# zhaowenlan1779/hekaton-system

Measured on AMD Instinct MI355X. Metric: subcircuit Groth16 proofs/sec (whole node), big-merkle, higher is better.
Workload: dtype u32 limbs (Montgomery mod-p integers)

## Files before the change

### __graft_entry__.py

```python
import os
import subprocess
import sys

ROOT = os.path.dirname(os.path.abspath(__file__))
if ROOT not in sys.path:
    sys.path.insert(0, ROOT)


def build():
    csrc = os.path.join(ROOT, "hekaton_system_amd", "csrc")
    jobs = str(min(8, os.cpu_count() or 1))
    subprocess.check_call(["make", "-C", csrc, "-j", jobs, "ARCH=gfx950"])
    subprocess.check_call(["make", "-C", csrc, "check", "ARCH=gfx950"], stdout=subprocess.DEVNULL)
    subprocess.check_call(["make", "-C", os.path.join(ROOT, "apps")], stdout=subprocess.DEVNULL)
    subprocess.check_call(["make", "-C", os.path.join(ROOT, "tests", "device_shim"), "-j", "2", "ARCH=gfx950"],
                          stdout=subprocess.DEVNULL)
    from oracle import c_oracle
    c_oracle.build()
    import hekaton_system_amd
    from hekaton_system_amd import capi
    lib = capi.load()
    for sym in capi.EXPORTS:
        getattr(lib, sym)


def smoke():
    import numpy as np
    from hekaton_system_amd import capi
    from tests import golden_util as gu
    case = gu.load("groth16.json")["bn254"][0]
    pk = case["pk"]
    with capi.Context("bn254", 0) as ctx:
        dpk = ctx.pk_upload(
            a_g=gu.hb(pk["a_g"]), b_g=gu.hb(pk["b_g"]), b_h=gu.hb(pk["b_h"]), h_g=gu.hb(pk["h_g"]),
            ck_stages=[gu.hb(c) for c in pk["ck"]], deltas_g=gu.hb(pk["deltas_g"]),
            last_delta_h=gu.hb(pk["last_delta_h"]), alpha_g=gu.hb(pk["alpha_g"]), beta_g=gu.hb(pk["beta_g"]),
            beta_h=gu.hb(pk["beta_h"]), matrices=(gu.csr(case["A"]), gu.csr(case["B"]), gu.csr(case["C"])),
            n_inst=case["n_inst"], n_constraints=case["n_constraints"])
        z = gu.hb(case["z_mont"])
        fr = ctx.fr_bytes
        s0, e0 = case["stage_ranges"][0]
        w0 = z[(case["n_inst"] + s0) * fr:(case["n_inst"] + e0) * fr]
        kap = gu.hb(case["kappas_mont"])
        com = dpk.commit(0, w0, kap[:fr])
        assert com.tobytes().hex() == case["comms"][0], "commitment differs from oracle"
        a, b, c = dpk.prove(z, gu.hb(case["r_mont"]), gu.hb(case["s_mont"]), kap)
        got = (a.tobytes().hex(), b.tobytes().hex(), c.tobytes().hex())
        want = (case["proof"]["a"], case["proof"]["b"], case["proof"]["c"])
        assert got == want, "proof differs from oracle"
        dpk.free()
    print("smoke ok: commit + prove on cuda:0 match the oracle bit for bit")


if __name__ == "__main__":
    build()
    print("build ok")
```

### hekaton_system_amd/csrc/ntt.cuh

```cuda
#pragma once
#include "field.cuh"

namespace hk {

constexpr int NTT_TILE_LOG = 11;
constexpr int NTT_THREADS = 512;
constexpr int POW_TABLE_BITS = 11;
constexpr int POW_TABLE_SIZE = 1 << POW_TABLE_BITS;

#if defined(__HIPCC__)

template <class Fr>
__device__ __forceinline__ Fr fr_load(const Fr* p) {
    Fr r;
    const uint4* s = reinterpret_cast<const uint4*>(p);
    uint4 a = s[0], b = s[1];
    r.v[0] = a.x; r.v[1] = a.y; r.v[2] = a.z; r.v[3] = a.w;
    r.v[4] = b.x; r.v[5] = b.y; r.v[6] = b.z; r.v[7] = b.w;
    return r;
}
template <class Fr>
__device__ __forceinline__ void fr_store(Fr* p, const Fr& lazy) {
    Fr r = Fr::canon(lazy);
    uint4* d = reinterpret_cast<uint4*>(p);
    d[0] = make_uint4(r.v[0], r.v[1], r.v[2], r.v[3]);
    d[1] = make_uint4(r.v[4], r.v[5], r.v[6], r.v[7]);
}

template <class Fr>
__global__ void k_pow_table(Fr* __restrict__ tw, const Fr* __restrict__ sq, u32 count, u32 nbits) {
    u32 i = blockIdx.x * blockDim.x + threadIdx.x;
    if (i >= count) return;
    Fr acc = Fr::one();
    for (u32 k = 0; k < nbits; k++)
        if ((i >> k) & 1) acc = Fr::mul(acc, fr_load(&sq[k]));
    fr_store(&tw[i], acc);
}

template <class Fr>
__device__ __forceinline__ Fr pow_from_tables(const Fr* __restrict__ pw, u32 j, u32 logn) {
    Fr g = fr_load(&pw[j & (POW_TABLE_SIZE - 1)]);
    if (logn > POW_TABLE_BITS) g = Fr::mul(g, fr_load(&pw[POW_TABLE_SIZE + ((j >> POW_TABLE_BITS) & (POW_TABLE_SIZE - 1))]));
    if (logn > 2 * POW_TABLE_BITS) g = Fr::mul(g, fr_load(&pw[2 * POW_TABLE_SIZE + (j >> (2 * POW_TABLE_BITS))]));
    return g;
}

template <class Fr>
__global__ void k_stage_tables(Fr* __restrict__ tws, const Fr* __restrict__ tw, u32 log_table) {
    size_t i = (size_t)blockIdx.x * blockDim.x + threadIdx.x;
    if ((i + 1) >> log_table) return;
    u32 s = 31 - __clz((u32)(i + 1));
    size_t j = i + 1 - ((size_t)1 << s);
    fr_store(&tws[i], fr_load(&tw[j << (log_table - s - 1)]));
}

template <class Fr, int DIT>
__global__ void __launch_bounds__(NTT_THREADS)
k_ntt_pass4(Fr* __restrict__ data, size_t stride_vec, const Fr* __restrict__ tws, u32 logn, u32 lo, u32 nst,
            u32 cols_bits, int post, u32 npost, Fr scale, const Fr* __restrict__ pw, const Fr* __restrict__ sub,
            Fr kc) {
    extern __shared__ uint4 lds_raw[];
    Fr* lds = reinterpret_cast<Fr*>(lds_raw);
    const u32 nthr = blockDim.x;
    if (blockIdx.y >= npost) post = 0;
    Fr* vec = data + (size_t)blockIdx.y * stride_vec;
    const u32 cols = 1u << cols_bits;
    const u32 tile_elems = 1u << (nst + cols_bits);
    const u32 mid_bits = lo - cols_bits;
    const u32 mid = blockIdx.x & ((1u << mid_bits) - 1u);
    const size_t base = ((size_t)(blockIdx.x >> mid_bits) << (lo + nst)) | ((size_t)mid << cols_bits);
    for (u32 e = threadIdx.x; e < tile_elems; e += nthr) {
        u32 r = e >> cols_bits, c = e & (cols - 1);
        lds[e] = fr_load(&vec[base | ((size_t)r << lo) | c]);
    }
    __syncthreads();
    const u32 npair = nst >> 1;
    for (u32 k = 0; k < npair; k++) {
        const u32 l = DIT ? 2 * k : nst - 2 - 2 * k;
        const u32 s = lo + l;
        const Fr* t_lo = tws + (((size_t)1 << s) - 1);
        const Fr* t_hi = tws + (((size_t)2 << s) - 1);
        for (u32 q = threadIdx.x; q < (tile_elems >> 2); q += nthr) {
            u32 c = q & (cols - 1), rr = q >> cols_bits;
            u32 r0 = ((rr >> l) << (l + 2)) | (rr & ((1u << l) - 1u));
            u32 j = (u32)((base | ((size_t)r0 << lo) | c) & (((size_t)1 << s) - 1));
            Fr wc = fr_load(&t_lo[j]);
            Fr wa = fr_load(&t_hi[j]);
            Fr wb = fr_load(&t_hi[j + (1u << s)]);
            u32 i0 = (r0 << cols_bits) | c, st = 1u << (l + cols_bits);
            Fr x0 = lds[i0], x1 = lds[i0 + st], x2 = lds[i0 + 2 * st], x3 = lds[i0 + 3 * st];
            if (DIT) {
                Fr v = Fr::mul(x1, wc), u = Fr::mul(x3, wc);
                x1 = Fr::sub(x0, v); x0 = Fr::add(x0, v);
                x3 = Fr::sub(x2, u); x2 = Fr::add(x2, u);
                v = Fr::mul(x2, wa); u = Fr::mul(x3, wb);
                x2 = Fr::sub(x0, v); x0 = Fr::add(x0, v);
                x3 = Fr::sub(x1, u); x1 = Fr::add(x1, u);
            } else {
                Fr v = Fr::sub(x0, x2), u = Fr::sub(x1, x3);
                x0 = Fr::add(x0, x2); x1 = Fr::add(x1, x3);
                x2 = Fr::mul(v, wa); x3 = Fr::mul(u, wb);
                v = Fr::sub(x0, x1); u = Fr::sub(x2, x3);
                x0 = Fr::add(x0, x1); x2 = Fr::add(x2, x3);
                x1 = Fr::mul(v, wc); x3 = Fr::mul(u, wc);
            }
            lds[i0] = x0; lds[i0 + st] = x1; lds[i0 + 2 * st] = x2; lds[i0 + 3 * st] = x3;
        }
        __syncthreads();
    }
    if (nst & 1) {
        const u32 l = DIT ? nst - 1 : 0;
        const u32 s = lo + l;
        const Fr* t_lo = tws + (((size_t)1 << s) - 1);
        for (u32 q = threadIdx.x; q < (tile_elems >> 1); q += nthr) {
            u32 c = q & (cols - 1), rr = q >> cols_bits;
            u32 r0 = ((rr >> l) << (l + 1)) | (rr & ((1u << l) - 1u));
            u32 j = (u32)((base | ((size_t)r0 << lo) | c) & (((size_t)1 << s) - 1));
            Fr w = fr_load(&t_lo[j]);
            u32 i0 = (r0 << cols_bits) | c, st = 1u << (l + cols_bits);
            Fr x0 = lds[i0], x1 = lds[i0 + st];
            if (DIT) {
                Fr v = Fr::mul(x1, w);
                lds[i0] = Fr::add(x0, v);
                lds[i0 + st] = Fr::sub(x0, v);
            } else {
                lds[i0] = Fr::add(x0, x1);
                lds[i0 + st] = Fr::mul(Fr::sub(x0, x1), w);
            }
        }
        __syncthreads();
    }
    for (u32 e = threadIdx.x; e < tile_elems; e += nthr) {
        u32 r = e >> cols_bits, c = e & (cols - 1);
        size_t gi = base | ((size_t)r << lo) | c;
        Fr x = lds[e];
        if (post & 2) x = Fr::mul(x, pow_from_tables(pw, logn ? (__brev((u32)gi) >> (32 - logn)) : 0u, logn));
        if (post & 4) x = Fr::sub(x, Fr::mul(fr_load(&sub[gi]), kc));
        if (post & 1) x = Fr::mul(x, scale);
        fr_store(&vec[gi], x);
    }
}

template <class Fr>
__global__ void k_scale_pow(Fr* __restrict__ data, size_t stride_vec, const Fr* __restrict__ pw, Fr scale,
                            u32 logn, int bitrev_index, int use_pow) {
    size_t pos = (size_t)blockIdx.x * blockDim.x + threadIdx.x;
    if (pos >> logn) return;
    Fr* vec = data + (size_t)blockIdx.y * stride_vec;
    Fr x = fr_load(&vec[pos]);
    x = Fr::mul(x, scale);
    if (use_pow) {
        u32 j = bitrev_index ? (logn ? (__brev((u32)pos) >> (32 - logn)) : 0u) : (u32)pos;
        x = Fr::mul(x, pow_from_tables(pw, j, logn));
    }
    fr_store(&vec[pos], x);
}

template <class Fr>
__global__ void k_bitrev(Fr* __restrict__ data, u32 logn) {
    size_t pos = (size_t)blockIdx.x * blockDim.x + threadIdx.x;
    if (pos >> logn) return;
    u32 r = logn ? (__brev((u32)pos) >> (32 - logn)) : 0u;
    if (r > pos) {
        Fr a = fr_load(&data[pos]), b = fr_load(&data[r]);
        fr_store(&data[pos], b);
        fr_store(&data[r], a);
    }
}

template <class Fr>
__global__ void k_mul_pointwise(Fr* __restrict__ a, const Fr* __restrict__ b, size_t m) {
    size_t i = (size_t)blockIdx.x * blockDim.x + threadIdx.x;
    if (i >= m) return;
    fr_store(&a[i], Fr::mul(fr_load(&a[i]), fr_load(&b[i])));
}

#endif

}
```

### hekaton_system_amd/csrc/ntt_host.cuh

```cuda
#pragma once
#include "curve_ops_impl.cuh"
#include "ntt.cuh"
#include "ntt_plan.h"
#include "csr.cuh"

namespace hk {

template <class Fr>
static Fr host_halve(const Fr& a) {
    u32 t[Fr::N + 1];
    u64 c = 0;
    bool odd = a.v[0] & 1;
    for (int i = 0; i < Fr::N; i++) {
        c += (u64)a.v[i] + (odd ? Fr::Params::MOD[i] : 0u);
        t[i] = (u32)c;
        c >>= 32;
    }
    t[Fr::N] = (u32)c;
    Fr r;
    for (int i = 0; i < Fr::N; i++) r.v[i] = (t[i] >> 1) | (t[i + 1] << 31);
    return r;
}
template <class Fr>
static Fr host_from_limbs(const u32* l) {
    Fr r;
    for (int i = 0; i < Fr::N; i++) r.v[i] = l[i];
    return r;
}

struct NttTables {
    std::mutex mu;
    u32 log_table = 0;
    void* tw_fwd = nullptr;
    void* tw_inv = nullptr;
    void* pw_g = nullptr;
    void* pw_ginv = nullptr;
    std::vector<void*> retired;
};

template <class C>
struct NttHost {
    typedef typename C::Fr Fr;

    static hk_status ensure(hk_ctx* ctx, u32 log_m, NttTables** out) {
        if (log_m > C::TWO_ADICITY) return HK_ERR_DOMAIN_TOO_LARGE;
        std::unique_lock<std::mutex> lk(ctx->mu);
        if (!ctx->ntt) ctx->ntt = new NttTables();
        NttTables* T = ctx->ntt;
        lk.unlock();
        std::unique_lock<std::mutex> tl(T->mu);
        *out = T;
        if (T->log_table >= log_m && T->tw_fwd) return HK_OK;
        u32 L = log_m < 16 ? 16 : log_m;
        if (L > C::TWO_ADICITY) L = C::TWO_ADICITY;
        HK_HIP(hipSetDevice(ctx->device));
        std::vector<Fr> sq(32), sqi(32);
        Fr w = host_from_limbs<Fr>(C::ROOT);
        for (u32 k = 0; k < C::TWO_ADICITY - L; k++) w = Fr::sqr(w);
        Fr winv = Fr::one();
        for (u32 k = 0; k < L; k++) {
            sq[k] = w;
            winv = Fr::mul(winv, w);
            w = Fr::sqr(w);
        }
        Fr t = winv;
        for (u32 k = 0; k < L; k++) { sqi[k] = t; t = Fr::sqr(t); }
        const u32 NG = 3 * POW_TABLE_BITS;
        std::vector<Fr> gs(NG), gis(NG);
        Fr g = host_from_limbs<Fr>(C::GEN), gi = host_from_limbs<Fr>(C::GEN_INV);
        for (u32 k = 0; k < NG; k++) { gs[k] = g; gis[k] = gi; g = Fr::sqr(g); gi = Fr::sqr(gi); }
        Fr *d_sq = nullptr, *tmp = nullptr, *tf = nullptr, *ti = nullptr, *pg = nullptr, *pgi = nullptr;
        size_t half = (size_t)1 << (L - 1), full = (size_t)1 << L;
        HK_HIP(hipMalloc((void**)&d_sq, sizeof(Fr) * (64 + 2 * NG)));
        HK_HIP(hipMalloc((void**)&tmp, sizeof(Fr) * half));
        HK_HIP(hipMalloc((void**)&tf, sizeof(Fr) * full));
        HK_HIP(hipMalloc((void**)&ti, sizeof(Fr) * full));
        HK_HIP(hipMalloc((void**)&pg, sizeof(Fr) * 3 * POW_TABLE_SIZE));
        HK_HIP(hipMalloc((void**)&pgi, sizeof(Fr) * 3 * POW_TABLE_SIZE));
        HK_HIP(hipMemcpy(d_sq, sq.data(), sizeof(Fr) * 32, hipMemcpyHostToDevice));
        HK_HIP(hipMemcpy(d_sq + 32, sqi.data(), sizeof(Fr) * 32, hipMemcpyHostToDevice));
        HK_HIP(hipMemcpy(d_sq + 64, gs.data(), sizeof(Fr) * NG, hipMemcpyHostToDevice));
        HK_HIP(hipMemcpy(d_sq + 64 + NG, gis.data(), sizeof(Fr) * NG, hipMemcpyHostToDevice));
        u32 blocks = (u32)((half + 255) / 256), blocks_full = (u32)((full + 255) / 256);
        hipLaunchKernelGGL((k_pow_table<Fr>), dim3(blocks), dim3(256), 0, 0, tmp, d_sq, (u32)half, L - 1);
        hipLaunchKernelGGL((k_stage_tables<Fr>), dim3(blocks_full), dim3(256), 0, 0, tf, tmp, L);
        hipLaunchKernelGGL((k_pow_table<Fr>), dim3(blocks), dim3(256), 0, 0, tmp, d_sq + 32, (u32)half, L - 1);
        hipLaunchKernelGGL((k_stage_tables<Fr>), dim3(blocks_full), dim3(256), 0, 0, ti, tmp, L);
        for (u32 lvl = 0; lvl < 3; lvl++) {
            hipLaunchKernelGGL((k_pow_table<Fr>), dim3(POW_TABLE_SIZE / 256), dim3(256), 0, 0, pg + POW_TABLE_SIZE * lvl,
                               d_sq + 64 + POW_TABLE_BITS * lvl, (u32)POW_TABLE_SIZE, (u32)POW_TABLE_BITS);
            hipLaunchKernelGGL((k_pow_table<Fr>), dim3(POW_TABLE_SIZE / 256), dim3(256), 0, 0, pgi + POW_TABLE_SIZE * lvl,
                               d_sq + 64 + NG + POW_TABLE_BITS * lvl, (u32)POW_TABLE_SIZE, (u32)POW_TABLE_BITS);
        }
        HK_HIP(hipGetLastError());
        HK_HIP(hipDeviceSynchronize());
        HK_HIP(hipFree(d_sq));
        HK_HIP(hipFree(tmp));
        for (void* p : {T->tw_fwd, T->tw_inv, T->pw_g, T->pw_ginv})
            if (p) T->retired.push_back(p);
        T->tw_fwd = tf; T->tw_inv = ti; T->pw_g = pg; T->pw_ginv = pgi;
        T->log_table = L;
        return HK_OK;
    }

    static Fr size_inv(u32 log_m) {
        Fr x = Fr::one();
        for (u32 k = 0; k < log_m; k++) x = host_halve(x);
        return x;
    }
    static Fr vanishing_inv_on_coset(u32 log_m) {
        Fr g = host_from_limbs<Fr>(C::GEN);
        for (u32 k = 0; k < log_m; k++) g = Fr::sqr(g);
        return fp_inv(Fr::sub(g, Fr::one()));
    }

    struct Post {
        int post = 0;
        u32 nvec = 0xffffffffu;
        const Fr* scale = nullptr;
        const Fr* pw = nullptr;
        const Fr* sub = nullptr;
        const Fr* kc = nullptr;
    };

    static hk_status passes(hipStream_t s, Fr* data, size_t stride, u32 batch, u32 logn, const Fr* tws, int dit,
                            const Post& ep = Post()) {
        if (logn == 0) return HK_OK;
        static const u32 tile_log = [] {
            const char* e = getenv("HK_NTT_TILE_LOG");
            return ntt_plan_tile_log(e ? (u32)atoi(e) : NTT_PLAN_TILE_LOG);
        }();
        static const u32 upper_max = [] {
            const char* e = getenv("HK_NTT_UPPER_MAX");
            return ntt_plan_upper_max(e ? (u32)atoi(e) : NTT_PLAN_UPPER_MAX, tile_log);
        }();
        const u32 threads = 1u << (tile_log - 2);
        NttPass ps[NTT_PLAN_MAX_PASSES];
        int np = ntt_pass_plan(logn, tile_log, upper_max, ps);
        Fr one = Fr::one();
        for (int k = 0; k < np; k++) {
            const NttPass& p = dit ? ps[k] : ps[np - 1 - k];
            u32 tile_log = p.nst + p.cols_bits;
            dim3 grid(1u << (logn - tile_log), batch);
            size_t lds = sizeof(Fr) << tile_log;
            bool last = k == np - 1;
            int pp = last ? ep.post : 0;
            const Fr& sc = (pp & 1) ? *ep.scale : one;
            const Fr& kc = (pp & 4) ? *ep.kc : one;
            if (dit)
                hipLaunchKernelGGL((k_ntt_pass4<Fr, 1>), grid, dim3(threads), lds, s, data, stride, tws, logn, p.lo,
                                   p.nst, p.cols_bits, pp, ep.nvec, sc, ep.pw, ep.sub, kc);
            else
                hipLaunchKernelGGL((k_ntt_pass4<Fr, 0>), grid, dim3(threads), lds, s, data, stride, tws, logn, p.lo,
                                   p.nst, p.cols_bits, pp, ep.nvec, sc, ep.pw, ep.sub, kc);
        }
        HK_HIP(hipGetLastError());
        return HK_OK;
    }

    static hk_status scale(hipStream_t s, Fr* data, size_t stride, u32 batch, u32 logn, const Fr* pw,
                           const Fr& sc, int bitrev_index, int use_pow) {
        size_t n = (size_t)1 << logn;
        hipLaunchKernelGGL((k_scale_pow<Fr>), dim3((u32)((n + 255) / 256), batch), dim3(256), 0, s, data,
                           stride, pw, sc, logn, bitrev_index, use_pow);
        HK_HIP(hipGetLastError());
        return HK_OK;
    }
    static hk_status bitrev(hipStream_t s, Fr* data, u32 logn) {
        size_t n = (size_t)1 << logn;
        hipLaunchKernelGGL((k_bitrev<Fr>), dim3((u32)((n + 255) / 256)), dim3(256), 0, s, data, logn);
        HK_HIP(hipGetLastError());
        return HK_OK;
    }
};

template <class C>
hk_status Ops<C>::ntt(hk_ctx* ctx, void* data, unsigned log_m, int inverse, int coset) {
    typedef NttHost<C> N;
    NttTables* T;
    HK_TRY(N::ensure(ctx, log_m, &T));
    LaneGuard g(ctx);
    Lane* L = g.lane;
    if (!L) return HK_ERR_DEVICE;
    size_t n = (size_t)1 << log_m;
    Fr* stage;
    HK_TRY(L->carve([&](Carve& c) { stage = c.n<Fr>(n); }));
    bool dev = is_device_ptr(data);
    Fr* d = (Fr*)data;
    if (!dev) {
        d = stage;
        HK_HIP(hipMemcpyAsync(d, data, n * sizeof(Fr), hipMemcpyHostToDevice, L->stream));
    }
    hipStream_t s = L->stream;
    if (!inverse) {
        if (coset) HK_TRY(N::scale(s, d, n, 1, log_m, (const Fr*)T->pw_g, Fr::one(), 0, 1));
        HK_TRY(N::passes(s, d, n, 1, log_m, (const Fr*)T->tw_fwd, 0));
        HK_TRY(N::bitrev(s, d, log_m));
    } else {
        Fr minv = N::size_inv(log_m);
        typename N::Post ep;
        ep.post = coset ? 3 : 1;
        ep.scale = &minv;
        ep.pw = (const Fr*)T->pw_ginv;
        HK_TRY(N::passes(s, d, n, 1, log_m, (const Fr*)T->tw_inv, 0, ep));
        HK_TRY(N::bitrev(s, d, log_m));
    }
    if (!dev) HK_HIP(hipMemcpyAsync(data, d, n * sizeof(Fr), hipMemcpyDeviceToHost, s));
    return L->settle();
}

template <class C>
struct QapHost {
    typedef typename C::Fr Fr;
    typedef NttHost<C> N;

    static u32 domain_log(size_t n_c, size_t n_inst) {
        size_t need = n_c + n_inst;
        u32 lg = 0;
        while (((size_t)1 << lg) < need) lg++;
        return lg;
    }
    static hk_status run(hipStream_t s, NttTables* T, const CsrDev& A, const CsrDev& B, const CsrDev& Cm,
                         size_t n_inst, size_t n_c, const Fr* z, Fr* abc, u32 log_m) {
        size_t m = (size_t)1 << log_m;
        const CsrDev* Ms[3] = {&A, &B, &Cm};
        for (int k = 0; k < 3; k++) {
            hipLaunchKernelGGL((k_spmv<Fr>), dim3((u32)((m + 255) / 256)), dim3(256), 0, s,
                               Ms[k]->row_ptr, Ms[k]->col, (const Fr*)Ms[k]->val, z, abc + k * m,
                               (u32)n_c, k == 0 ? (u32)n_inst : 0u, (u32)m);
        }
        const Fr* tinv = (const Fr*)T->tw_inv;
        const Fr* tfwd = (const Fr*)T->tw_fwd;
        typename N::Post e1;
        e1.post = 2;
        e1.nvec = 2;
        e1.pw = (const Fr*)T->pw_g;
        HK_TRY(N::passes(s, abc, m, 3, log_m, tinv, 0, e1));
        HK_TRY(N::passes(s, abc, m, 2, log_m, tfwd, 1));
        hipLaunchKernelGGL((k_mul_pointwise<Fr>), dim3((u32)((m + 255) / 256)), dim3(256), 0, s, abc, abc + m, m);
        Fr minv = N::size_inv(log_m);
        Fr mm = fp_inv(Fr::mul(minv, minv));
        Fr k = Fr::mul(N::vanishing_inv_on_coset(log_m), Fr::mul(minv, Fr::mul(minv, minv)));
        typename N::Post e2;
        e2.post = 2 | 4 | 1;
        e2.pw = (const Fr*)T->pw_ginv;
        e2.sub = abc + 2 * m;
        e2.kc = &mm;
        e2.scale = &k;
        HK_TRY(N::passes(s, abc, m, 1, log_m, tinv, 0, e2));
        HK_HIP(hipGetLastError());
        return HK_OK;
    }
};

template <class C>
hk_status Ops<C>::witness_map(hk_ctx* ctx, const hk_csr* A, const hk_csr* B, const hk_csr* Cm, size_t n_inst,
                              size_t n_c, const void* z, size_t n_v, void* h_out, size_t h_cap,
                              size_t* m_out) {
    typedef QapHost<C> Q;
    if (A->n_rows != n_c || B->n_rows != n_c || Cm->n_rows != n_c || n_inst > n_v || n_inst < 1) return HK_ERR_ARG;
    if (!csr_host_ok(A) || !csr_host_ok(B) || !csr_host_ok(Cm)) return HK_ERR_ARG;
    u32 log_m = Q::domain_log(n_c, n_inst);
    if (log_m > C::TWO_ADICITY) return HK_ERR_DOMAIN_TOO_LARGE;
    size_t m = (size_t)1 << log_m;
    if (m_out) *m_out = m;
    if (h_cap < m) return HK_ERR_LEN;
    NttTables* T;
    HK_TRY(NttHost<C>::ensure(ctx, log_m, &T));
    R1csStage stage(A, B, Cm, n_v, sizeof(Fr));
    Staged zin = staged(z, n_v * sizeof(Fr));
    LaneGuard g(ctx);
    Lane* L = g.lane;
    if (!L) return HK_ERR_DEVICE;
    Fr* abc;
    HK_TRY(L->carve([&](Carve& c) {
        stage.carve(c);
        stage_carve(c, &zin, 1);
        abc = c.n<Fr>(3 * m);
    }));
    CsrDev D[3];
    HK_TRY(stage.upload(L, D));
    HK_TRY(stage_upload(L, &zin, 1));
    HK_TRY(Q::run(L->stream, T, D[0], D[1], D[2], n_inst, n_c, (const Fr*)zin.p, abc, log_m));
    HK_TRY(NttHost<C>::bitrev(L->stream, abc, log_m));
    HK_HIP(hipMemcpyAsync(h_out, abc, m * sizeof(Fr),
                          is_device_ptr(h_out) ? hipMemcpyDeviceToDevice : hipMemcpyDeviceToHost, L->stream));
    return L->settle();
}

template <class C>
void Ops<C>::ctx_release(hk_ctx* ctx) {
    for (auto& e : ctx->fb_cache)
        if (e.table) (void)hipFree(e.table);
    ctx->fb_cache.clear();
    if (!ctx->ntt) return;
    NttTables* T = ctx->ntt;
    for (void* p : {T->tw_fwd, T->tw_inv, T->pw_g, T->pw_ginv})
        if (p) (void)hipFree(p);
    for (void* p : T->retired) (void)hipFree(p);
    delete T;
    ctx->ntt = nullptr;
}

}
```

Baseline: 126.3.

## Precompute coset twist tables and special-case trivial-twiddle NTT stages

Adds cached per-size coset twist tables in bit-reversed order. The post-NTT coset multiply becomes a single table load instead of up to three pow-table loads and two multiplies, and the quotient scale is folded into the inverse table and the subtraction constant. It also reorders the odd radix-2 stage and adds specialised s==0 radix-4/radix-2 butterflies that skip twiddle loads and multiplies by one. The trade-offs are two extra m-sized device tables per domain size, a one-time build with a stream sync, and more branching in the NTT kernel.

```diff
diff --git a/__graft_entry__.py b/__graft_entry__.py
--- a/__graft_entry__.py
+++ b/__graft_entry__.py
@@ -15,6 +15,8 @@
     subprocess.check_call(["make", "-C", os.path.join(ROOT, "apps")], stdout=subprocess.DEVNULL)
     subprocess.check_call(["make", "-C", os.path.join(ROOT, "tests", "device_shim"), "-j", "2", "ARCH=gfx950"],
                           stdout=subprocess.DEVNULL)
+    subprocess.check_call(["make", "-C", os.path.join(ROOT, "tests", "device_shim"), "-f", "twist.mk", "-j", "2",
+                           "ARCH=gfx950"], stdout=subprocess.DEVNULL)
     from oracle import c_oracle
     c_oracle.build()
     import hekaton_system_amd
diff --git a/hekaton_system_amd/csrc/ntt.cuh b/hekaton_system_amd/csrc/ntt.cuh
--- a/hekaton_system_amd/csrc/ntt.cuh
+++ b/hekaton_system_amd/csrc/ntt.cuh
@@ -52,6 +52,14 @@
     u32 s = 31 - __clz((u32)(i + 1));
     size_t j = i + 1 - ((size_t)1 << s);
     fr_store(&tws[i], fr_load(&tw[j << (log_table - s - 1)]));
+}
+
+template <class Fr>
+__global__ void k_twist_table(Fr* __restrict__ out, const Fr* __restrict__ pw, Fr c, u32 logn) {
+    size_t i = (size_t)blockIdx.x * blockDim.x + threadIdx.x;
+    if (i >> logn) return;
+    u32 j = logn ? (__brev((u32)i) >> (32 - logn)) : 0u;
+    fr_store(&out[i], Fr::mul(pow_from_tables(pw, j, logn), c));
 }
 
 template <class Fr, int DIT>
@@ -74,12 +82,65 @@
         lds[e] = fr_load(&vec[base | ((size_t)r << lo) | c]);
     }
     __syncthreads();
-    const u32 npair = nst >> 1;
-    for (u32 k = 0; k < npair; k++) {
-        const u32 l = DIT ? 2 * k : nst - 2 - 2 * k;
+    const u32 npair = nst >> 1, odd = nst & 1;
+    const u32 lone = odd ? ((!DIT && lo == 0) ? 0u : npair) : 0xffffffffu;
+    for (u32 t = 0; t < npair + odd; t++) {
+        if (t == lone) {
+            const u32 l = (DIT || lo == 0) ? nst - 1 : 0;
+            const u32 s = lo + l;
+            const Fr* t_lo = tws + (((size_t)1 << s) - 1);
+            for (u32 q = threadIdx.x; q < (tile_elems >> 1); q += nthr) {
+                u32 c = q & (cols - 1), rr = q >> cols_bits;
+                u32 r0 = ((rr >> l) << (l + 1)) | (rr & ((1u << l) - 1u));
+                u32 i0 = (r0 << cols_bits) | c, st = 1u << (l + cols_bits);
+                if (s == 0) {
+                    Fr x0 = lds[i0], x1 = lds[i0 + st];
+                    lds[i0] = Fr::add(x0, x1);
+                    lds[i0 + st] = Fr::sub(x0, x1);
+                    continue;
+                }
+                u32 j = (u32)((base | ((size_t)r0 << lo) | c) & (((size_t)1 << s) - 1));
+                Fr w = fr_load(&t_lo[j]);
+                Fr x0 = lds[i0], x1 = lds[i0 + st];
+                if (DIT) {
+                    Fr v = Fr::mul(x1, w);
+                    lds[i0] = Fr::add(x0, v);
+                    lds[i0 + st] = Fr::sub(x0, v);
+                } else {
+                    lds[i0] = Fr::add(x0, x1);
+                    lds[i0 + st] = Fr::mul(Fr::sub(x0, x1), w);
+                }
+            }
+            __syncthreads();
+            continue;
+        }
+        const u32 k = t - (lone == 0 ? 1u : 0u);
+        const u32 l = DIT ? 2 * k : 2 * (npair - 1 - k) + ((odd && lo != 0) ? 1u : 0u);
         const u32 s = lo + l;
         const Fr* t_lo = tws + (((size_t)1 << s) - 1);
         const Fr* t_hi = tws + (((size_t)2 << s) - 1);
+        if (s == 0) {
+            const Fr wb = fr_load(&t_hi[1]);
+            for (u32 q = threadIdx.x; q < (tile_elems >> 2); q += nthr) {
+                u32 i0 = q << 2;
+                Fr x0 = lds[i0], x1 = lds[i0 + 1], x2 = lds[i0 + 2], x3 = lds[i0 + 3];
+                if (DIT) {
+                    Fr v = Fr::add(x0, x1), u = Fr::add(x2, x3);
+                    x1 = Fr::sub(x0, x1);
+                    x3 = Fr::mul(Fr::sub(x2, x3), wb);
+                    x0 = Fr::add(v, u); x2 = Fr::sub(v, u);
+                    v = Fr::add(x1, x3); x3 = Fr::sub(x1, x3); x1 = v;
+                } else {
+                    Fr v = Fr::sub(x0, x2), u = Fr::mul(Fr::sub(x1, x3), wb);
+                    x0 = Fr::add(x0, x2); x1 = Fr::add(x1, x3);
+                    x2 = Fr::add(v, u); x3 = Fr::sub(v, u);
+                    v = Fr::sub(x0, x1); x0 = Fr::add(x0, x1); x1 = v;
+                }
+                lds[i0] = x0; lds[i0 + 1] = x1; lds[i0 + 2] = x2; lds[i0 + 3] = x3;
+            }
+            __syncthreads();
+            continue;
+        }
         for (u32 q = threadIdx.x; q < (tile_elems >> 2); q += nthr) {
             u32 c = q & (cols - 1), rr = q >> cols_bits;
             u32 r0 = ((rr >> l) << (l + 2)) | (rr & ((1u << l) - 1u));
@@ -108,33 +169,12 @@
         }
         __syncthreads();
     }
-    if (nst & 1) {
-        const u32 l = DIT ? nst - 1 : 0;
-        const u32 s = lo + l;
-        const Fr* t_lo = tws + (((size_t)1 << s) - 1);
-        for (u32 q = threadIdx.x; q < (tile_elems >> 1); q += nthr) {
-            u32 c = q & (cols - 1), rr = q >> cols_bits;
-            u32 r0 = ((rr >> l) << (l + 1)) | (rr & ((1u << l) - 1u));
-            u32 j = (u32)((base | ((size_t)r0 << lo) | c) & (((size_t)1 << s) - 1));
-            Fr w = fr_load(&t_lo[j]);
-            u32 i0 = (r0 << cols_bits) | c, st = 1u << (l + cols_bits);
-            Fr x0 = lds[i0], x1 = lds[i0 + st];
-            if (DIT) {
-                Fr v = Fr::mul(x1, w);
-                lds[i0] = Fr::add(x0, v);
-                lds[i0 + st] = Fr::sub(x0, v);
-            } else {
-                lds[i0] = Fr::add(x0, x1);
-                lds[i0 + st] = Fr::mul(Fr::sub(x0, x1), w);
-            }
-        }
-        __syncthreads();
-    }
     for (u32 e = threadIdx.x; e < tile_elems; e += nthr) {
         u32 r = e >> cols_bits, c = e & (cols - 1);
         size_t gi = base | ((size_t)r << lo) | c;
         Fr x = lds[e];
         if (post & 2) x = Fr::mul(x, pow_from_tables(pw, logn ? (__brev((u32)gi) >> (32 - logn)) : 0u, logn));
+        if (post & 8) x = Fr::mul(x, fr_load(&pw[gi]));
         if (post & 4) x = Fr::sub(x, Fr::mul(fr_load(&sub[gi]), kc));
         if (post & 1) x = Fr::mul(x, scale);
         fr_store(&vec[gi], x);
diff --git a/hekaton_system_amd/csrc/ntt_host.cuh b/hekaton_system_amd/csrc/ntt_host.cuh
--- a/hekaton_system_amd/csrc/ntt_host.cuh
+++ b/hekaton_system_amd/csrc/ntt_host.cuh
@@ -1,4 +1,5 @@
 #pragma once
+#include <map>
 #include "curve_ops_impl.cuh"
 #include "ntt.cuh"
 #include "ntt_plan.h"
@@ -36,6 +37,11 @@
     void* pw_g = nullptr;
     void* pw_ginv = nullptr;
     std::vector<void*> retired;
+    struct Twist {
+        void* fwd = nullptr;
+        void* inv = nullptr;
+    };
+    std::map<u32, Twist> twist;
 };
 
 template <class C>
@@ -112,6 +118,48 @@
         Fr g = host_from_limbs<Fr>(C::GEN);
         for (u32 k = 0; k < log_m; k++) g = Fr::sqr(g);
         return fp_inv(Fr::sub(g, Fr::one()));
+    }
+
+    static Fr quotient_scale(u32 log_m) {
+        Fr minv = size_inv(log_m);
+        return Fr::mul(vanishing_inv_on_coset(log_m), Fr::mul(minv, Fr::mul(minv, minv)));
+    }
+
+    static bool twist_enabled() {
+        static const bool on = [] {
+            const char* e = getenv("HK_NTT_TWIST_TABLE");
+            return !(e && atoi(e) == 0);
+        }();
+        return on;
+    }
+
+    static hk_status twist(NttTables* T, u32 log_m, const Fr** fwd, const Fr** inv) {
+        std::unique_lock<std::mutex> tl(T->mu);
+        NttTables::Twist& tw = T->twist[log_m];
+        if (!tw.inv) {
+            size_t m = (size_t)1 << log_m;
+            Fr *f = nullptr, *b = nullptr;
+            HK_HIP(hipMalloc((void**)&f, sizeof(Fr) * m));
+            hipError_t e = hipMalloc((void**)&b, sizeof(Fr) * m);
+            if (e == hipSuccess) {
+                dim3 grid((u32)((m + 255) / 256));
+                hipLaunchKernelGGL((k_twist_table<Fr>), grid, dim3(256), 0, 0, f, (const Fr*)T->pw_g, Fr::one(), log_m);
+                hipLaunchKernelGGL((k_twist_table<Fr>), grid, dim3(256), 0, 0, b, (const Fr*)T->pw_ginv,
+                                   quotient_scale(log_m), log_m);
+                e = hipGetLastError();
+                if (e == hipSuccess) e = hipStreamSynchronize(0);
+            }
+            if (e != hipSuccess) {
+                (void)hipFree(f);
+                if (b) (void)hipFree(b);
+                HK_HIP(e);
+            }
+            tw.fwd = f;
+            tw.inv = b;
+        }
+        *fwd = (const Fr*)tw.fwd;
+        *inv = (const Fr*)tw.inv;
+        return HK_OK;
     }
 
     struct Post {
@@ -231,21 +279,25 @@
         }
         const Fr* tinv = (const Fr*)T->tw_inv;
         const Fr* tfwd = (const Fr*)T->tw_fwd;
+        const bool folded = N::twist_enabled();
+        const Fr *gf = nullptr, *gb = nullptr;
+        if (folded) HK_TRY(N::twist(T, log_m, &gf, &gb));
         typename N::Post e1;
-        e1.post = 2;
+        e1.post = folded ? 8 : 2;
         e1.nvec = 2;
-        e1.pw = (const Fr*)T->pw_g;
+        e1.pw = folded ? gf : (const Fr*)T->pw_g;
         HK_TRY(N::passes(s, abc, m, 3, log_m, tinv, 0, e1));
         HK_TRY(N::passes(s, abc, m, 2, log_m, tfwd, 1));
         hipLaunchKernelGGL((k_mul_pointwise<Fr>), dim3((u32)((m + 255) / 256)), dim3(256), 0, s, abc, abc + m, m);
         Fr minv = N::size_inv(log_m);
         Fr mm = fp_inv(Fr::mul(minv, minv));
-        Fr k = Fr::mul(N::vanishing_inv_on_coset(log_m), Fr::mul(minv, Fr::mul(minv, minv)));
+        Fr k = N::quotient_scale(log_m);
+        Fr kmm = Fr::mul(k, mm);
         typename N::Post e2;
-        e2.post = 2 | 4 | 1;
-        e2.pw = (const Fr*)T->pw_ginv;
+        e2.post = folded ? (8 | 4) : (2 | 4 | 1);
+        e2.pw = folded ? gb : (const Fr*)T->pw_ginv;
         e2.sub = abc + 2 * m;
-        e2.kc = &mm;
+        e2.kc = folded ? &kmm : &mm;
         e2.scale = &k;
         HK_TRY(N::passes(s, abc, m, 1, log_m, tinv, 0, e2));
         HK_HIP(hipGetLastError());
@@ -298,6 +350,9 @@
     for (void* p : {T->tw_fwd, T->tw_inv, T->pw_g, T->pw_ginv})
         if (p) (void)hipFree(p);
     for (void* p : T->retired) (void)hipFree(p);
+    for (auto& kv : T->twist)
+        for (void* p : {kv.second.fwd, kv.second.inv})
+            if (p) (void)hipFree(p);
     delete T;
     ctx->ntt = nullptr;
 }
```

New measurement: 128.4, median of 6. 1.02x the previous value.
